# mathisbot/homomorph-rust

Measured on AMD Instinct MI355X. Metric: homomorphic u32 ops/sec (add, mul) at d=dp=tau=128; 1/2/4/8 MI355X, higher is better.
Workload: dtype u32

## Files before the change

homomorph-rust_amd/csrc/adder.hip:

```cpp
#include <hip/hip_runtime.h>

#include "dev_common.h"

namespace hm {


__device__ __forceinline__ uint32_t limb_off(const Bounds &B, uint32_t i) {
    uint32_t o = 0;
    for (uint32_t j = 0; j < i; ++j) o += cap_of(B.b[j]);
    return o;
}

__device__ __forceinline__ uint64_t checked_limb(uint64_t v, uint32_t d, uint32_t bnd, uint32_t k, bool &bad) {
    const uint32_t nl = d / 64 + 1;
    if (d > bnd) {
        bad = true;
        return 0;
    }
    if (k >= nl) {
        bad |= v != 0;
        return 0;
    }
    if (k == nl - 1) {
        const uint32_t top = d % 64;
        const uint64_t keep = (~0ull) >> (63 - top);
        bad |= (v & ~keep) != 0;
        v &= keep;
        if (d > 0 && !((v >> top) & 1ull)) bad = true;
    }
    return v;
}

__device__ __forceinline__ void stage_ab(const uint64_t *__restrict__ pa, const uint32_t *__restrict__ da,
                                         const Bounds &BA, const uint64_t *__restrict__ pb,
                                         const uint32_t *__restrict__ db, const Bounds &BB, uint32_t i0,
                                         uint32_t nb, uint32_t *Al, uint32_t cntA, uint32_t *nAl,
                                         uint32_t *Bl, uint32_t cntB, uint32_t *nBl, uint32_t *tb,
                                         int *status, uint32_t bmask = ~0u) {
    const uint32_t lane = (uint32_t)lane_id();
    i0 = rfl(i0), nb = rfl(nb);
    pa += limb_off(BA, i0), pb += limb_off(BB, i0);
    da += i0, db += i0;
    uint32_t dga = 0, dgb = 0;
    if (lane < nb) dga = da[lane], dgb = db[lane];
    uint32_t tota = 0, totb = 0, vba = 0, vea = 0, vbb = 0, veb = 0;
    for (uint32_t t = 0; t < nb; ++t) {
        const uint32_t j = (i0 + t) & bmask;
        const uint32_t ba = BA.b[j], bb = BB.b[j];
        tota += cap_of(ba), totb += cap_of(bb);
        if (lane == t) vba = ba, vea = tota, vbb = bb, veb = totb;
    }
    const uint64_t fa = lane < tota ? pa[lane] : 0ull, fb = lane < totb ? pb[lane] : 0ull;
    uint32_t *bnda = tb, *enda = tb + nb, *bndb = tb + 2 * nb, *endb = tb + 3 * nb;
    if (lane < nb) {
        bnda[lane] = vba, enda[lane] = vea, bndb[lane] = vbb, endb[lane] = veb;
        nAl[lane] = dga, nBl[lane] = dgb;
    }
    for (uint32_t k = lane; k < nb * cntA; k += kWave) Al[k] = 0u;
    for (uint32_t k = lane; k < nb * cntB; k += kWave) Bl[k] = 0u;
    wsync();
    bool bad = false;
    auto one = [&](const uint64_t *src, uint64_t first, uint32_t total, const uint32_t *bnd,
                   const uint32_t *ends, const uint32_t *deg, uint32_t *dst, uint32_t cnt) {
        uint32_t t = 0, lo = 0, hi = nb ? ends[0] : 0;
        for (uint32_t g = lane; g < total; g += kWave) {
            while (g >= hi) ++t, lo = hi, hi = ends[t];
            const uint32_t k = g - lo;
            const uint64_t v = checked_limb(g == lane ? first : src[g], deg[t], bnd[t], k, bad);
            dst[t * cnt + 2 * k] = (uint32_t)v;
            dst[t * cnt + 2 * k + 1] = (uint32_t)(v >> 32);
        }
    };
    one(pa, fa, tota, bnda, enda, nAl, Al, cntA);
    one(pb, fb, totb, bndb, endb, nBl, Bl, cntB);
    if (__any(bad) && lane == 0) flag(status, HM_ERR_BAD_INPUT);
    wsync();
    if (lane < nb) {
        const uint32_t d1 = nAl[lane], d2 = nBl[lane];
        uint32_t n1 = d1 / 32 + 1, n2 = d2 / 32 + 1;
        if (d1 > bnda[lane] || (d1 == 0 && !(Al[lane * cntA] & 1u))) n1 = 0;
        if (d2 > bndb[lane] || (d2 == 0 && !(Bl[lane * cntB] & 1u))) n2 = 0;
        nAl[lane] = n1, nBl[lane] = n2;
    }
}

template <int NB, int NAB, bool TOP1 = false, bool MULTI = false>
__global__ void __launch_bounds__(256) add_prep_kernel(AddArgs A) {
    extern __shared__ uint32_t lds[];
    const uint32_t wave = rfl(threadIdx.x >> 6);
    const uint64_t gw = (uint64_t)blockIdx.x * (blockDim.x >> 6) + wave;
    const int lane = lane_id();
    const uint32_t L = A.nbits;
    uint64_t e;
    uint32_t bpw, i0, nmine;
    if constexpr (MULTI) {
        e = gw * A.vpw;
        if (e >= A.n) return;
        bpw = A.vpw * L;
        i0 = 0;
        nmine = (uint32_t)min((uint64_t)A.vpw, A.n - e) * L;
    } else {
        e = gw / A.wpv;
        const uint32_t part = (uint32_t)(gw % A.wpv);
        if (e >= A.n) return;
        bpw = (L + A.wpv - 1) / A.wpv;
        i0 = min(L, part * bpw), nmine = min(L, i0 + bpw) - i0;
    }
    auto val_of = [&](uint32_t t) -> uint32_t { return MULTI ? t >> A.lgL : 0u; };
    auto bit_of = [&](uint32_t t) -> uint32_t { return MULTI ? t & (L - 1) : i0 + t; };
    uint32_t *Ls = lds + (size_t)wave * A.prep_lds;
    uint32_t *Al = Ls, *Bl = Al + bpw * A.cntA, *Xl = Bl + bpw * A.cntB;
    uint32_t *ABl = Xl + bpw * A.cntX, *Pl = ABl + bpw * A.cntAB;
    uint32_t *nAl = Pl + bpw * A.cntP, *nBl = nAl + bpw, *dAB = nBl + bpw, *dP = dAB + bpw;
    const size_t oP = (size_t)L * A.cntAB, oDA = oP + (size_t)L * A.cntP, oDP = oDA + L, oX = oDP + L;
    uint32_t *ws = A.ws + e * A.ws_stride;
    auto wsv = [&](uint32_t t) { return MULTI ? ws + (size_t)val_of(t) * A.ws_stride : ws; };
    const uint64_t *pa = A.a.limbs + e * A.a.stride, *pb = A.b.limbs + e * A.b.stride;
    const uint32_t *da = A.a.degree + e * L, *db = A.b.degree + e * L;

    stage_ab(pa, da, A.ab, pb, db, A.bb, i0, nmine, Al, A.cntA, nAl, Bl, A.cntB, nBl, dAB, A.status,
             MULTI ? L - 1 : ~0u);
    for (uint32_t k = lane; k < 2 * bpw; k += kWave) dAB[k] = 0u;
    wsync();
    const uint32_t nprod = MULTI ? nmine : min(nmine, (L - 1) - min(i0, L - 1));
    auto has_prod = [&](uint32_t t) { return !MULTI || bit_of(t) + 1 < L; };

    for (uint32_t f = lane; f < nmine * A.cntX; f += kWave) {
        const uint32_t t = f / A.cntX, m = f % A.cntX, i = bit_of(t);
        const int na = (int)nAl[t], nb = (int)nBl[t];
        const uint32_t x = ((int)m < na ? Al[t * A.cntA + m] : 0u) ^
                           ((int)m < nb ? Bl[t * A.cntB + m] : 0u);
        Xl[t * A.cntX + m] = x;
        wsv(t)[oX + (size_t)i * A.cntX + m] = x;
    }

    const uint32_t cq = A.cntX - (TOP1 ? 1u : 0u);
    const uint32_t qt = A.cntX - 1;
    auto top_rows = [&](uint32_t cnt, auto &&len, auto &&set, const uint32_t *src, uint32_t scnt,
                        uint32_t *dst, uint32_t dcnt) {
        const uint32_t dt = kWave / cnt, dk = kWave % cnt;
        uint32_t t = (uint32_t)lane / cnt, k = (uint32_t)lane % cnt;
        for (uint32_t f0 = 0; f0 < nprod * cnt; f0 += kWave) {
            if (t < nprod && has_prod(t) && k < len(t) && set(t))
                atomicXor(&dst[t * dcnt + qt + k], src[t * scnt + k]);
            t += dt, k += dk;
            if (k >= cnt) k -= cnt, ++t;
        }
    };
    auto for_rows = [&](auto &&row) {
        const uint32_t dt = kWave / cq, dq = kWave % cq;
        uint32_t t = (uint32_t)lane / cq, q = (uint32_t)lane % cq;
        for (uint32_t f0 = 0; f0 < nprod * cq; f0 += kWave) {
            if (t < nprod && has_prod(t)) row(t, q);
            t += dt, q += dq;
            if (q >= cq) q -= cq, ++t;
        }
    };
    for (uint32_t k = lane; k < nprod * A.cntAB; k += kWave) ABl[k] = 0u;
    for (uint32_t k = lane; k < nprod * A.cntP; k += kWave) Pl[k] = 0u;
    wsync();
    for_rows([&](uint32_t t, uint32_t q) {
        if ((int)q < (int)nAl[t]) {
            if constexpr (NB > 0) {
                if (nBl[t]) clmul_row_xor_fixed<NB>(Al[t * A.cntA + q], Bl + t * NB, ABl + t * NAB + q);
            } else {
                clmul_row_xor(Al[t * A.cntA + q], Bl + t * A.cntB, (int)nBl[t], ABl + t * A.cntAB + q);
            }
        }
    });
    if constexpr (TOP1)
        top_rows(A.cntB, [&](uint32_t t) { return nBl[t]; }, [&](uint32_t t) { return nAl[t] == A.cntX; },
                 Bl, A.cntB, ABl, A.cntAB);
    wsync();
    for (uint32_t f = lane; f < nprod * A.cntAB; f += kWave) {
        const uint32_t t = f / A.cntAB, m = f % A.cntAB;
        const uint32_t w = ABl[f];
        if (has_prod(t)) wsv(t)[(size_t)bit_of(t) * A.cntAB + m] = w;
        if (w) atomicMax(&dAB[t], m * 32 + 32 - __builtin_clz(w));
    }
    wsync();
    for_rows([&](uint32_t t, uint32_t q) {
        const int nx = max((int)nAl[t], (int)nBl[t]);
        if ((int)q < nx) {
            if constexpr (NAB > 0) {
                if (dAB[t]) clmul_row_xor_fixed<NAB>(Xl[t * A.cntX + q], ABl + t * NAB, Pl + t * A.cntP + q);
            } else {
                clmul_row_xor(Xl[t * A.cntX + q], ABl + t * A.cntAB, bitwords((int)dAB[t]),
                              Pl + t * A.cntP + q);
            }
        }
    });
    if constexpr (TOP1)
        top_rows(A.cntAB, [&](uint32_t t) { return (uint32_t)bitwords((int)dAB[t]); },
                 [&](uint32_t t) { return (Xl[t * A.cntX + qt] & 1u) != 0; }, ABl, A.cntAB, Pl, A.cntP);
    wsync();
    for (uint32_t f = lane; f < nprod * A.cntP; f += kWave) {
        const uint32_t t = f / A.cntP, m = f % A.cntP;
        const uint32_t w = Pl[f] ^ (m < A.cntX ? Xl[t * A.cntX + m] : 0u);
        if (has_prod(t)) wsv(t)[oP + (size_t)bit_of(t) * A.cntP + m] = w;
        if (w) atomicMax(&dP[t], m * 32 + 32 - __builtin_clz(w));
    }
    wsync();
    for (uint32_t t = lane; t < nprod; t += kWave) {
        if (!has_prod(t)) continue;
        const uint32_t i = bit_of(t);
        wsv(t)[oDA + i] = dAB[t];
        wsv(t)[oDP + i] = dP[t];
    }
}

template <int CAP>
__global__ void __launch_bounds__(256) add_prep_uniform_kernel(AddArgs A) {
    constexpr uint32_t kBound = 64u * (CAP - 1);
    constexpr uint32_t cA = 2 * CAP, cX = 2 * CAP - 1, cAB = 4 * CAP - 3, cP = 6 * CAP - 5;
    constexpr uint32_t cq = cX - 1, qt = cX - 1;
    extern __shared__ uint32_t lds[];
    const uint32_t wave = rfl(threadIdx.x >> 6);
    const uint64_t gw = (uint64_t)blockIdx.x * (blockDim.x >> 6) + wave;
    const uint32_t lane = (uint32_t)lane_id();
    const uint32_t L = A.nbits;
    uint64_t e;
    uint32_t part;
    if ((gw >> 32) == 0)
        e = (uint32_t)gw / A.wpv, part = (uint32_t)gw % A.wpv;
    else
        e = gw / A.wpv, part = (uint32_t)(gw % A.wpv);
    if (e >= A.n) return;
    const uint32_t bpw = (L + A.wpv - 1) / A.wpv;
    const uint32_t i0 = rfl(min(L, part * bpw)), nmine = rfl(min(L, i0 + bpw) - i0);
    const uint32_t nprod = rfl(min(nmine, (L - 1) - min(i0, L - 1)));
    auto lanes = [&](uint32_t n, auto &&body) {
        for (uint32_t f0 = 0; f0 < n; f0 += kWave)
            if (f0 + lane < n) body(f0 + lane);
    };
    uint32_t *Ls = lds + (size_t)wave * A.prep_lds;
    uint32_t *Al = Ls, *Bl = Al + bpw * cA, *Xl = Bl + bpw * cA;
    uint32_t *ABl = Xl + bpw * cX, *Pl = ABl + bpw * cAB;
    uint32_t *nAl = Pl + bpw * cP, *nBl = nAl + bpw, *nXl = nBl + bpw, *nABl = nXl + bpw;
    uint32_t *dXl = nABl + bpw;
    const size_t oP = (size_t)L * cAB, oDA = oP + (size_t)L * cP, oDP = oDA + L, oX = oDP + L;
    uint32_t *ws = A.ws + e * A.ws_stride;
    const uint64_t *pa = A.a.limbs + e * A.a.stride + (size_t)i0 * CAP;
    const uint64_t *pb = A.b.limbs + e * A.b.stride + (size_t)i0 * CAP;
    const uint32_t *da = A.a.degree + e * L + i0, *db = A.b.degree + e * L + i0;

    uint32_t dga = 0, dgb = 0;
    if (lane < nmine) dga = da[lane], dgb = db[lane];
    const uint32_t tot = nmine * CAP;
    uint64_t fa[2], fb[2];
#pragma unroll
    for (uint32_t j = 0; j < 2; ++j) {
        const uint32_t g = lane + j * kWave;
        fa[j] = g < tot ? pa[g] : 0ull, fb[j] = g < tot ? pb[g] : 0ull;
    }
    lanes(nprod * cAB, [&](uint32_t f) { ABl[f] = 0u; });
    constexpr uint32_t cPz = cP - cX;
    lanes(nprod * cPz, [&](uint32_t f) { Pl[f / cPz * cP + cX + f % cPz] = 0u; });
    if (lane < nmine) nAl[lane] = dga, nBl[lane] = dgb, dXl[lane] = 0u;
    wsync();
    bool bad = false;
    auto stage = [&](uint32_t g, uint64_t va, uint64_t vb) {
        const uint32_t t = g / CAP, k = g % CAP;
        va = checked_limb(va, nAl[t], kBound, k, bad);
        vb = checked_limb(vb, nBl[t], kBound, k, bad);
        *(uint2 *)(Al + t * cA + 2 * k) = make_uint2((uint32_t)va, (uint32_t)(va >> 32));
        *(uint2 *)(Bl + t * cA + 2 * k) = make_uint2((uint32_t)vb, (uint32_t)(vb >> 32));
        const uint64_t x = va ^ vb;
        const uint32_t xl = (uint32_t)x, xh = (uint32_t)(x >> 32);
        uint32_t *xs = Xl + t * cX + 2 * k, *xg = ws + oX + (size_t)(i0 + t) * cX + 2 * k;
        uint32_t *xp = Pl + t * cP + 2 * k;
        const bool prod = t < nprod;
        xs[0] = xl, xg[0] = xl;
        if (prod) xp[0] = xl;
        if (k + 1 < CAP) {
            xs[1] = xh, xg[1] = xh;
            if (prod) xp[1] = xh;
        }
        if (x) atomicMax(&dXl[t], 64 * k + 64 - (uint32_t)__builtin_clzll(x));
    };
#pragma unroll
    for (uint32_t j = 0; j < 2; ++j)
        if (lane + j * kWave < tot) stage(lane + j * kWave, fa[j], fb[j]);
    for (uint32_t g0 = 2 * kWave; g0 < tot; g0 += kWave)
        if (g0 + lane < tot) stage(g0 + lane, pa[g0 + lane], pb[g0 + lane]);
    if (__any(bad) && lane == 0) flag(A.status, HM_ERR_BAD_INPUT);
    wsync();
    if (lane < nmine) {
        uint32_t a1 = dga + 1, b1 = dgb + 1;
        if (dga > kBound || (dga == 0 && !(Al[lane * cA] & 1u))) a1 = 0;
        if (dgb > kBound || (dgb == 0 && !(Bl[lane * cA] & 1u))) b1 = 0;
        const uint32_t x1 = dXl[lane];
        const uint32_t ab1 = a1 && b1 ? a1 + b1 - 1 : 0u;
        const uint32_t p1 = !x1 ? 0u : !ab1 ? x1 : x1 + ab1 - 1;
        nAl[lane] = (uint32_t)bitwords((int)a1), nBl[lane] = (uint32_t)bitwords((int)b1);
        nXl[lane] = (uint32_t)bitwords((int)x1), nABl[lane] = (uint32_t)bitwords((int)ab1);
        if (lane < nprod) ws[oDA + i0 + lane] = ab1, ws[oDP + i0 + lane] = p1;
    }
    wsync();
    lanes(nprod * cq, [&](uint32_t f) {
        const uint32_t t = f / cq, q = f % cq;
        if (q < nAl[t]) clmul_row_xor(Al[t * cA + q], Bl + t * cA, (int)nBl[t], ABl + t * cAB + q);
    });
    lanes(nprod * cA, [&](uint32_t f) {
        const uint32_t t = f / cA, k = f % cA;
        if (k < nBl[t] && nAl[t] == cX) atomicXor(&ABl[t * cAB + qt + k], Bl[f]);
    });
    wsync();
    uint32_t *wsab = ws + (size_t)i0 * cAB, *wsp = ws + oP + (size_t)i0 * cP;
    lanes(nprod * cAB, [&](uint32_t f) {
        const uint32_t t = f / cAB, k = f % cAB;
        const uint32_t w = ABl[f];
        wsab[f] = w;
        if (k < nABl[t] && (Xl[t * cX + qt] & 1u)) atomicXor(&Pl[t * cP + qt + k], w);
    });
    lanes(nprod * cq, [&](uint32_t f) {
        const uint32_t t = f / cq, q = f % cq;
        if (q < nXl[t]) clmul_row_xor(Xl[t * cX + q], ABl + t * cAB, (int)nABl[t], Pl + t * cP + q);
    });
    wsync();
    lanes(nprod * cP, [&](uint32_t f) { wsp[f] = Pl[f]; });
}

__device__ __forceinline__ int store_sum_bit(const uint64_t *pa, uint32_t dga, const uint64_t *pb, uint32_t dgb,
                             const uint32_t *C, int nc, uint64_t *__restrict__ dst, uint32_t bound,
                             uint32_t *deg_out, int *status) {
    const int lane = lane_id();
    const int cap = (int)cap_of(bound);
    const int nla = (int)(dga >> 6) + 1, nlb = (int)(dgb >> 6) + 1;
    const uint64_t ma = (~0ull) >> (63 - (dga & 63)), mb = (~0ull) >> (63 - (dgb & 63));
    const int total = max(max(cap, max(nla, nlb)), (nc + 1) / 2);
    int ldeg = -1;
    for (int g = lane; g < total; g += kWave) {
        uint64_t v = 0;
        if (g < nla) v ^= g == nla - 1 ? (pa[g] & ma) : pa[g];
        if (g < nlb) v ^= g == nlb - 1 ? (pb[g] & mb) : pb[g];
        const int w = 2 * g;
        const uint32_t lo = w < nc ? C[w] : 0u, hi = w + 1 < nc ? C[w + 1] : 0u;
        v ^= (uint64_t)lo | ((uint64_t)hi << 32);
        if (g < cap) dst[g] = v;
        if (v) ldeg = g * 64 + 63 - __builtin_clzll(v);
    }
    const int deg = wave_max_i32(ldeg);
    if (lane == 0) {
        if (deg > (int)bound) flag(status, HM_ERR_CAPACITY);
        *deg_out = (uint32_t)max(deg, 0);
    }
    return deg;
}

template <int WMAX, bool PAD>
__global__ void __launch_bounds__(256) add_chain_kernel(AddArgs A) {
    kt_start(A.kt);
    extern __shared__ uint32_t lds[];
    const int wave = (int)rfl(threadIdx.x >> 6);
    const uint64_t e = (uint64_t)blockIdx.x * (blockDim.x >> 6) + wave;
    if (e >= A.n) {
        kt_finish(A.kt);
        return;
    }
    const int lane = lane_id();
    const uint32_t L = A.nbits;
    uint32_t *Ls = lds + (size_t)wave * A.chain_lds;
    uint32_t *C = Ls + kHalo, *Cn = C + A.cw + kHalo;
    uint32_t *Pl = Cn + A.cw;
    const uint32_t *ws = A.ws + e * A.ws_stride;
    const uint32_t *ABg = ws, *Pg = ws + (size_t)L * A.cntAB;
    const uint32_t *degABg = Pg + (size_t)L * A.cntP, *degPg = degABg + L;
    const uint64_t *pa = A.a.limbs + e * A.a.stride, *pb = A.b.limbs + e * A.b.stride;
    uint64_t *po = A.out.limbs + e * A.out.stride;
    const uint32_t *da = A.a.degree + e * L, *db = A.b.degree + e * L;
    uint32_t *dout = A.out.degree + e * L;

    const uint32_t ncarry = 2 * (A.cw + kHalo);
    for (uint32_t k = lane; k < ncarry; k += kWave) Ls[k] = 0u;
    for (uint32_t k = lane; k < (L - 1) * A.cntP; k += kWave) Pl[k] = Pg[k];
    wsync();
    int nc = 0;
    uint32_t offa = 0, offb = 0, offo = 0;
    for (uint32_t i = 0; i < L; ++i) {
        store_sum_bit(pa + offa, rfl(da[i]), pb + offb, rfl(db[i]), C, nc, po + offo, A.ob.b[i],
                      dout + i, A.status);
        if (i + 1 < L) {
            const int np = bitwords((int)degPg[i]), nab = bitwords((int)degABg[i]);
            int nout;
            nc = words_of(wave_mul<kQBig, WMAX, PAD>(Pl + (size_t)i * A.cntP, np, C, nc,
                                                     ABg + (size_t)i * A.cntAB, nab, Cn, &nout));
            wsync();
            uint32_t *t = C;
            C = Cn;
            Cn = t;
        }
        offa += cap_of(A.ab.b[i]);
        offb += cap_of(A.bb.b[i]);
        offo += cap_of(A.ob.b[i]);
    }
    kt_finish(A.kt);
}

template <int WMAX>
__global__ void __launch_bounds__(256) add_chain_staged_kernel(AddArgs A) {
    kt_start(A.kt);
    extern __shared__ uint32_t lds[];
    const int wave = (int)rfl(threadIdx.x >> 6);
    const uint64_t e = (uint64_t)blockIdx.x * (blockDim.x >> 6) + wave;
    if (e >= A.n) {
        kt_finish(A.kt);
        return;
    }
    const int lane = lane_id();
    const uint32_t L = A.nbits;
    uint32_t *Ls = lds + (size_t)wave * A.chain_lds;
    uint32_t *C = Ls + kHalo;
    uint32_t *Pl = C + A.cw, *ABl = Pl + (size_t)(L - 1) * A.cntP;
    uint32_t *Xl = ABl + (size_t)(L - 1) * A.cntAB, *dPl = Xl + (size_t)L * A.cntX, *dABl = dPl + L;
    const uint32_t *ws = A.ws + e * A.ws_stride;
    const uint32_t *ABg = ws, *Pg = ws + (size_t)L * A.cntAB;
    const uint32_t *degABg = Pg + (size_t)L * A.cntP, *degPg = degABg + L, *Xg = degPg + L;
    uint64_t *po = A.out.limbs + e * A.out.stride;
    uint32_t *dout = A.out.degree + e * L;

    for (uint32_t k = lane; k < kHalo + A.cw; k += kWave) Ls[k] = 0u;
    for (uint32_t k = lane; k < (L - 1) * A.cntP; k += kWave) Pl[k] = Pg[k];
    for (uint32_t k = lane; k < (L - 1) * A.cntAB; k += kWave) ABl[k] = ABg[k];
    for (uint32_t k = lane; k < L * A.cntX; k += kWave) Xl[k] = Xg[k];
    for (uint32_t k = lane; k < L; k += kWave) dPl[k] = degPg[k], dABl[k] = degABg[k];
    wsync();
    int nc = 0;
    uint32_t offo = 0;
    for (uint32_t i = 0; i < L; ++i) {
        store_sum_x(Xl + (size_t)i * A.cntX, (int)A.cntX, C, nc, po + offo, A.ob.b[i], dout + i,
                    A.status);
        if (i + 1 < L) {
            const int np = bitwords((int)rfl(dPl[i])), nab = bitwords((int)rfl(dABl[i]));
            int nout;
            wsync();
            nc = words_of(wave_mul<kQBig, WMAX, true>(Pl + (size_t)i * A.cntP, np, C, nc,
                                                      ABl + (size_t)i * A.cntAB, nab, C, &nout));
            wsync();
        }
        offo += cap_of(A.ob.b[i]);
    }
    kt_finish(A.kt);
}

int launch_add_prep(const AddArgs &a, void *stream) {
    if (a.n == 0) return 0;
    const uint64_t waves = a.vpw > 1 ? (a.n + a.vpw - 1) / a.vpw : a.n * a.wpv;
    const uint64_t blocks = (waves + 3) / 4;
    const size_t lds = (size_t)a.prep_lds * 4 * 4;
#ifndef HM_PREP_FIXED
#define HM_PREP_FIXED 0
#endif
    if (a.ucap == 5 && a.vpw <= 1)
        hipLaunchKernelGGL((add_prep_uniform_kernel<5>), dim3((unsigned)blocks), dim3(256), lds, (hipStream_t)stream, a);
    else if (a.ucap)
        return -1;
    else if (a.vpw > 1 && a.top1)
        hipLaunchKernelGGL((add_prep_kernel<0, 0, true, true>), dim3((unsigned)blocks), dim3(256), lds, (hipStream_t)stream, a);
    else if (a.vpw > 1)
        hipLaunchKernelGGL((add_prep_kernel<0, 0, false, true>), dim3((unsigned)blocks), dim3(256), lds, (hipStream_t)stream, a);
    else if (a.top1)
        hipLaunchKernelGGL((add_prep_kernel<0, 0, true>), dim3((unsigned)blocks), dim3(256), lds, (hipStream_t)stream, a);
    else if (HM_PREP_FIXED && a.cntB == 10 && a.cntAB == 17)
        hipLaunchKernelGGL((add_prep_kernel<10, 17>), dim3((unsigned)blocks), dim3(256), lds, (hipStream_t)stream, a);
    else if (HM_PREP_FIXED && a.cntB == 6 && a.cntAB == 9)
        hipLaunchKernelGGL((add_prep_kernel<6, 9>), dim3((unsigned)blocks), dim3(256), lds, (hipStream_t)stream, a);
    else if (HM_PREP_FIXED && a.cntB == 18 && a.cntAB == 33)
        hipLaunchKernelGGL((add_prep_kernel<18, 33>), dim3((unsigned)blocks), dim3(256), lds, (hipStream_t)stream, a);
    else
        hipLaunchKernelGGL((add_prep_kernel<0, 0>), dim3((unsigned)blocks), dim3(256), lds, (hipStream_t)stream, a);
    return hipGetLastError() == hipSuccess ? 0 : -1;
}

AddArgs add_args_slice(const AddArgs &a, uint64_t e0, uint64_t n) {
    AddArgs s = a;
    s.a.limbs += e0 * a.a.stride, s.a.degree += e0 * a.a.dstride;
    s.b.limbs += e0 * a.b.stride, s.b.degree += e0 * a.b.dstride;
    s.out.limbs += e0 * a.out.stride, s.out.degree += e0 * a.out.dstride;
    s.ws += e0 * a.ws_stride;
    s.n = n;
    return s;
}

int launch_add(const AddArgs &a, void *stream) {
    if (a.n == 0) return 0;
    if (launch_add_prep(a, stream)) return -1;
    return a.mfma ? launch_add_chain_mfma(a, stream) : launch_add_chain_valu(a, stream);
}

int launch_add_chain_valu(const AddArgs &a, void *stream) {
    const int wpb = kAddWavesPerBlock;
    const uint64_t blocks = (a.n + wpb - 1) / wpb;
    const size_t lds = (size_t)a.chain_lds * 4 * wpb;
    const uint32_t need = (a.max_prod_words + 63) / 64;
    const bool pad = a.pad != 0;
#define HM_LAUNCH_ADD(WM)                                                                         \
    do {                                                                                          \
        if (a.staged)                                                                             \
            hipLaunchKernelGGL((add_chain_staged_kernel<WM>), dim3((unsigned)blocks),             \
                               dim3(64 * wpb), lds, (hipStream_t)stream, a);                      \
        else if (pad)                                                                             \
            hipLaunchKernelGGL((add_chain_kernel<WM, true>), dim3((unsigned)blocks),              \
                               dim3(64 * wpb), lds, (hipStream_t)stream, a);                      \
        else                                                                                      \
            hipLaunchKernelGGL((add_chain_kernel<WM, false>), dim3((unsigned)blocks),             \
                               dim3(64 * wpb), lds, (hipStream_t)stream, a);                      \
    } while (0)
    if (need <= 4) HM_LAUNCH_ADD(4);
    else if (need <= 8) HM_LAUNCH_ADD(8);
    else if (need <= 12) HM_LAUNCH_ADD(12);
    else if (need <= 16) HM_LAUNCH_ADD(16);
    else HM_LAUNCH_ADD(24);
#undef HM_LAUNCH_ADD
    return hipGetLastError() == hipSuccess ? 0 : -1;
}

}
```

homomorph-rust_amd/csrc/dev_common.h:

```cpp
#pragma once
#include <hip/hip_runtime.h>

#include "engine.h"
#include "gf2_wave.h"

namespace hm {

__device__ __forceinline__ void flag(int *status, int code) {
    if (status) atomicCAS(status, 0, code);
}

__device__ __forceinline__ void wsync() {
    __builtin_amdgcn_fence(__ATOMIC_RELEASE, "wavefront");
    __builtin_amdgcn_wave_barrier();
    __builtin_amdgcn_fence(__ATOMIC_ACQUIRE, "wavefront");
}
__device__ __forceinline__ void gsync() {
    __builtin_amdgcn_fence(__ATOMIC_RELEASE, "workgroup");
    __builtin_amdgcn_wave_barrier();
    __builtin_amdgcn_fence(__ATOMIC_ACQUIRE, "workgroup");
}


__device__ __forceinline__ void arg_to_lds(const uint32_t (&a)[HM_MAX_BITS], uint32_t n, uint32_t *lds) {
    static_assert(HM_MAX_BITS % 16 == 0, "whole 16-entry chunks");
    n = rfl(n);
    const bool l0 = (threadIdx.x & 63u) == 0;
    for (uint32_t c = 0; c < n; c += 16) {
        uint32_t v[16];
#pragma unroll
        for (int j = 0; j < 16; ++j) v[j] = a[c + j];
        if (l0) {
            uint4 *d = (uint4 *)(lds + c);
#pragma unroll
            for (int q = 0; q < 4; ++q) d[q] = make_uint4(v[4 * q], v[4 * q + 1], v[4 * q + 2], v[4 * q + 3]);
        }
    }
}

__device__ __forceinline__ int load_bit(const uint64_t *__restrict__ src, uint32_t deg, uint32_t bound,
                        uint32_t *__restrict__ dst, int *status) {
    const int lane = lane_id();
    if (deg > bound) {
        if (lane == 0) flag(status, HM_ERR_BAD_INPUT);
        return 0;
    }
    const int nl = (int)(deg / 64) + 1;
    const int cap = (int)(bound / 64) + 1;
    const uint32_t tb = deg % 64;
    bool bad = false;
    for (int g = lane; g < cap; g += kWave) {
        uint64_t v = src[g];
        if (g >= nl) {
            bad |= v != 0;
            continue;
        }
        if (g == nl - 1) {
            const uint64_t keep = (~0ull) >> (63 - tb);
            bad |= (v & ~keep) != 0;
            v &= keep;
            if (deg > 0 && !((v >> tb) & 1ull)) bad = true;
        }
        dst[2 * g] = (uint32_t)v;
        dst[2 * g + 1] = (uint32_t)(v >> 32);
    }
    if (__any(bad) && lane == 0) flag(status, HM_ERR_BAD_INPUT);
    if (deg == 0) {
        const uint32_t w0 = rfl((uint32_t)src[0]);
        if (!(w0 & 1u)) return 0;
    }
    return (int)(deg / 32) + 1;
}

__device__ __forceinline__ int store_xor_bit(const uint32_t *X, int nx, const uint32_t *C, int nc,
                             uint64_t *__restrict__ dst, uint32_t bound, uint32_t *deg_out,
                             int *status) {
    const int lane = lane_id();
    const int cap = (int)cap_of(bound);
    const int n = max(nx, nc);
    const int total = max(cap, (n + 1) / 2);
    int ldeg = -1;
    for (int g = lane; g < total; g += kWave) {
        const int w = 2 * g;
        uint32_t lo = (w < nx ? X[w] : 0u) ^ (w < nc ? C[w] : 0u);
        uint32_t hi = (w + 1 < nx ? X[w + 1] : 0u) ^ (w + 1 < nc ? C[w + 1] : 0u);
        uint64_t v = (uint64_t)lo | ((uint64_t)hi << 32);
        if (g < cap) dst[g] = v;
        if (v) ldeg = g * 64 + 63 - __builtin_clzll(v);
    }
    const int deg = wave_max_i32(ldeg);
    if (lane == 0) {
        if (deg > (int)bound) flag(status, HM_ERR_CAPACITY);
        *deg_out = (uint32_t)max(deg, 0);
    }
    return deg;
}

struct WaveSlice {
    uint64_t e;
    uint32_t *lds;
    bool live;
};
__device__ __forceinline__ WaveSlice wave_slice(uint32_t *lds, uint32_t lds_per_wave, uint64_t n) {
    const int wave = (int)rfl(threadIdx.x >> 6);
    const uint64_t e = (uint64_t)blockIdx.x * (blockDim.x >> 6) + wave;
    return {e, lds + (size_t)wave * lds_per_wave, e < n};
}

struct BitReader {
    const uint64_t *limbs;
    const uint32_t *degree;
    uint32_t off = 0;
    int *status;
    __device__ __forceinline__ BitReader(const BatchArg &x, uint64_t e, int *status)
        : limbs(x.limbs + e * x.stride), degree(x.degree + e * x.dstride), status(status) {}
    __device__ __forceinline__ int load(uint32_t i, uint32_t bound, uint32_t *dst) {
        const int n = load_bit(limbs + off, rfl(degree[i]), bound, dst, status);
        off += cap_of(bound);
        return n;
    }
    __device__ __forceinline__ int load_down(uint32_t i, uint32_t bound, uint32_t *dst) {
        off -= cap_of(bound);
        return load_bit(limbs + off, rfl(degree[i]), bound, dst, status);
    }
};
struct BitWriter {
    uint64_t *limbs;
    uint32_t *degree;
    uint32_t off = 0;
    int *status;
    __device__ __forceinline__ BitWriter(const BatchArg &x, uint64_t e, int *status)
        : limbs(x.limbs + e * x.stride), degree(x.degree + e * x.dstride), status(status) {}
    __device__ __forceinline__ void store(uint32_t i, uint32_t bound, const uint32_t *X, int nx,
                                          const uint32_t *C = nullptr, int nc = 0) {
        store_xor_bit(X, nx, C, nc, limbs + off, bound, degree + i, status);
        off += cap_of(bound);
    }
};

__device__ __forceinline__ int store_sum_x(const uint32_t *X, int nx, const uint32_t *C, int nc,
                           uint64_t *__restrict__ dst, uint32_t bound, uint32_t *deg_out,
                           int *status) {
    const int lane = lane_id();
    const int cap = (int)cap_of(bound);
    const int total = max(cap, (max(nx, nc) + 1) / 2);
    int ldeg = -1;
    for (int g = lane; g < total; g += kWave) {
        const int w = 2 * g;
        const uint32_t lo = (w < nx ? X[w] : 0u) ^ (w < nc ? C[w] : 0u);
        const uint32_t hi = (w + 1 < nx ? X[w + 1] : 0u) ^ (w + 1 < nc ? C[w + 1] : 0u);
        const uint64_t v = (uint64_t)lo | ((uint64_t)hi << 32);
        if (g < cap) dst[g] = v;
        if (v) ldeg = g * 64 + 63 - __builtin_clzll(v);
    }
    const int deg = wave_max_i32(ldeg);
    if (lane == 0) {
        if (deg > (int)bound) flag(status, HM_ERR_CAPACITY);
        *deg_out = (uint32_t)max(deg, 0);
    }
    return deg;
}

__device__ __forceinline__ int words_of(int deg) { return deg >= 0 ? nwords(deg) : 0; }

__device__ __forceinline__ int store_xor3_bit(const uint32_t *Aw, int na, const uint32_t *Bw, int nb,
                              const uint32_t *C, int nc, uint64_t *__restrict__ dst,
                              uint32_t bound, uint32_t *deg_out, int *status) {
    const int lane = lane_id();
    const int cap = (int)cap_of(bound);
    const int n = max(max(na, nb), nc);
    const int total = max(cap, (n + 1) / 2);
    int ldeg = -1;
    for (int g = lane; g < total; g += kWave) {
        const int w = 2 * g;
        uint32_t lo = (w < na ? Aw[w] : 0u) ^ (w < nb ? Bw[w] : 0u) ^ (w < nc ? C[w] : 0u);
        uint32_t hi = (w + 1 < na ? Aw[w + 1] : 0u) ^ (w + 1 < nb ? Bw[w + 1] : 0u) ^
                      (w + 1 < nc ? C[w + 1] : 0u);
        uint64_t v = (uint64_t)lo | ((uint64_t)hi << 32);
        if (g < cap) dst[g] = v;
        if (v) ldeg = g * 64 + 63 - __builtin_clzll(v);
    }
    const int deg = wave_max_i32(ldeg);
    if (lane == 0) {
        if (deg > (int)bound) flag(status, HM_ERR_CAPACITY);
        *deg_out = (uint32_t)max(deg, 0);
    }
    return deg;
}

constexpr int kQSmall = 10;
constexpr int kQBig = 25;

struct Holey {
    uint32_t h[4];
    __device__ __forceinline__ explicit Holey(uint32_t v) {
#pragma unroll
        for (int a = 0; a < 4; ++a) h[a] = v & (0x11111111u << a);
    }
};

__device__ __forceinline__ void holey_acc(uint32_t z[4], const Holey &U, const Holey &V1,
                                          const Holey &V0) {
#pragma unroll
    for (int c = 0; c < 4; ++c) {
        uint32_t lo[4], hi[4];
#pragma unroll
        for (int a = 0; a < 4; ++a) {
            const int b = (c - a) & 3;
            lo[a] = U.h[a] * V1.h[b];
            hi[a] = __umulhi(U.h[a], V0.h[b]);
        }
        z[c] = __builtin_amdgcn_bitop3_b32(__builtin_amdgcn_bitop3_b32(z[c], lo[0], lo[1], 0x96),
                                           __builtin_amdgcn_bitop3_b32(lo[2], lo[3], hi[0], 0x96),
                                           __builtin_amdgcn_bitop3_b32(hi[1], hi[2], hi[3], 0x96), 0x96);
    }
}

__device__ __forceinline__ uint32_t xor4(uint32_t a, uint32_t b, uint32_t c, uint32_t d) {
    return __builtin_amdgcn_bitop3_b32(a, b, c, 0x96) ^ d;
}

__device__ __forceinline__ uint32_t holey_fold(const uint32_t z[4]) {
    return (z[0] & 0x11111111u) | (z[1] & 0x22222222u) | (z[2] & 0x44444444u) |
           (z[3] & 0x88888888u);
}

__device__ __forceinline__ uint32_t clmul_word(const uint32_t *__restrict__ pu, int nu,
                                               const uint32_t *__restrict__ pv, int nv, int m) {
    uint32_t z[4] = {0u, 0u, 0u, 0u};
    const int qlo = max(0, m - nv), qhi = min(nu - 1, m);
    if (qlo > qhi) return 0u;
    int k = m - qlo;
    Holey V1(k < nv ? pv[k] : 0u);
    for (int q = qlo; q <= qhi; ++q, --k) {
        const Holey V0((k >= 1 && k - 1 < nv) ? pv[k - 1] : 0u);
        holey_acc(z, Holey(pu[q]), V1, V0);
        V1 = V0;
    }
    return holey_fold(z);
}

__device__ __forceinline__ void clmul_row_xor(uint32_t u, const uint32_t *__restrict__ pv, int nv,
                                              uint32_t *out) {
    const Holey U(u);
    uint32_t hiprev = 0u;
#ifndef HM_CLMUL_PEEL
#define HM_CLMUL_PEEL 1
#endif
    if (HM_CLMUL_PEEL) {
        if (nv <= 0) return;
        uint32_t vnext = pv[0];
        for (int k = 0; k < nv; ++k) {
            const Holey V(vnext);
            vnext = pv[min(k + 1, nv - 1)];
            uint32_t zl[4], zh[4];
#pragma unroll
            for (int c = 0; c < 4; ++c) {
                uint64_t p[4];
#pragma unroll
                for (int a = 0; a < 4; ++a) p[a] = (uint64_t)U.h[a] * V.h[(c - a) & 3];
                zl[c] = xor4((uint32_t)p[0], (uint32_t)p[1], (uint32_t)p[2], (uint32_t)p[3]);
                zh[c] = xor4((uint32_t)(p[0] >> 32), (uint32_t)(p[1] >> 32), (uint32_t)(p[2] >> 32),
                             (uint32_t)(p[3] >> 32));
            }
            atomicXor(&out[k], holey_fold(zl) ^ hiprev);
            hiprev = holey_fold(zh);
        }
        if (hiprev) atomicXor(&out[nv], hiprev);
        return;
    }
    uint32_t vnext = nv > 0 ? pv[0] : 0u;
    for (int k = 0; k <= nv; ++k) {
        uint32_t lo = 0u, hi = 0u;
        if (k < nv) {
            const Holey V(vnext);
            vnext = k + 1 < nv ? pv[k + 1] : 0u;
            uint32_t zl[4], zh[4];
#pragma unroll
            for (int c = 0; c < 4; ++c) {
                uint64_t p[4];
#pragma unroll
                for (int a = 0; a < 4; ++a) p[a] = (uint64_t)U.h[a] * V.h[(c - a) & 3];
                zl[c] = xor4((uint32_t)p[0], (uint32_t)p[1], (uint32_t)p[2], (uint32_t)p[3]);
                zh[c] = xor4((uint32_t)(p[0] >> 32), (uint32_t)(p[1] >> 32), (uint32_t)(p[2] >> 32),
                             (uint32_t)(p[3] >> 32));
            }
            lo = holey_fold(zl), hi = holey_fold(zh);
        }
        const uint32_t w = lo ^ hiprev;
        if (w) atomicXor(&out[k], w);
        hiprev = hi;
    }
}

template <int NV>
__device__ __forceinline__ void clmul_row_xor_fixed(uint32_t u, const uint32_t *__restrict__ pv,
                                                    uint32_t *out) {
    const Holey U(u);
    uint32_t v[NV];
#pragma unroll
    for (int k = 0; k < NV; ++k) v[k] = pv[k];
    uint32_t hiprev = 0u;
#pragma unroll
    for (int k = 0; k < NV; ++k) {
        const Holey V(v[k]);
        uint32_t zl[4], zh[4];
#pragma unroll
        for (int c = 0; c < 4; ++c) {
            uint64_t p[4];
#pragma unroll
            for (int a = 0; a < 4; ++a) p[a] = (uint64_t)U.h[a] * V.h[(c - a) & 3];
            zl[c] = xor4((uint32_t)p[0], (uint32_t)p[1], (uint32_t)p[2], (uint32_t)p[3]);
            zh[c] = xor4((uint32_t)(p[0] >> 32), (uint32_t)(p[1] >> 32), (uint32_t)(p[2] >> 32),
                         (uint32_t)(p[3] >> 32));
        }
        atomicXor(&out[k], holey_fold(zl) ^ hiprev);
        hiprev = holey_fold(zh);
    }
    if (hiprev) atomicXor(&out[NV], hiprev);
}

__device__ __forceinline__ uint32_t kt_wave() {
    return (blockIdx.x * ((blockDim.x + 63u) >> 6) + (threadIdx.x >> 6)) & (kTimerWaves - 1);
}
__device__ __forceinline__ void kt_start(const KTimer &k) {
    if (k.t0 && (threadIdx.x & 63u) == 0)
        __hip_atomic_fetch_min(&k.t0[kt_wave()], (unsigned long long)wall_clock64(),
                               __ATOMIC_RELAXED, __HIP_MEMORY_SCOPE_AGENT);
}
__device__ __forceinline__ void kt_finish(const KTimer &k) {
    if (k.t1 && (threadIdx.x & 63u) == 0)
        __hip_atomic_fetch_max(&k.t1[kt_wave()], (unsigned long long)wall_clock64(),
                               __ATOMIC_RELAXED, __HIP_MEMORY_SCOPE_AGENT);
}

__device__ __forceinline__ int bitwords(int degp1) { return degp1 ? ((degp1 - 1) >> 5) + 1 : 0; }

}
```

Before: 9.828 million.

## Pair holey-multiply products and peel monic top words from GF(2) clmul rows

Restructures the carry-less multiply core so some pairs of holey sub-products are summed with one integer add before extraction. Static checks confirm no 4-bit field overflows, cutting the XOR count, and folding uses bitop3 bit-select with masks held opaque in VGPRs. In the polynomial product kernel, the known-monic leading word of each operand is handled with direct XORs of the other operand's words instead of full clmul rows, shortening row lengths. This adds constexpr bookkeeping and relies on the leading-word-equals-one invariant for correctness.

```diff
diff --git a/homomorph-rust_amd/csrc/adder.hip b/homomorph-rust_amd/csrc/adder.hip
--- a/homomorph-rust_amd/csrc/adder.hip
+++ b/homomorph-rust_amd/csrc/adder.hip
@@ -299,23 +299,31 @@
     wsync();
     lanes(nprod * cq, [&](uint32_t f) {
         const uint32_t t = f / cq, q = f % cq;
-        if (q < nAl[t]) clmul_row_xor(Al[t * cA + q], Bl + t * cA, (int)nBl[t], ABl + t * cAB + q);
+        if (q < nAl[t])
+            clmul_row_xor(Al[t * cA + q], Bl + t * cA, (int)min(nBl[t], qt), ABl + t * cAB + q);
     });
     lanes(nprod * cA, [&](uint32_t f) {
         const uint32_t t = f / cA, k = f % cA;
-        if (k < nBl[t] && nAl[t] == cX) atomicXor(&ABl[t * cAB + qt + k], Bl[f]);
+        const uint32_t w = (nAl[t] == cX && k < cX ? Bl[f] : 0u) ^ (nBl[t] == cX && k < qt ? Al[f] : 0u);
+        if (w) atomicXor(&ABl[t * cAB + qt + k], w);
     });
     wsync();
+    constexpr uint32_t qtab = cAB - 1;
     uint32_t *wsab = ws + (size_t)i0 * cAB, *wsp = ws + oP + (size_t)i0 * cP;
     lanes(nprod * cAB, [&](uint32_t f) {
         const uint32_t t = f / cAB, k = f % cAB;
         const uint32_t w = ABl[f];
         wsab[f] = w;
         if (k < nABl[t] && (Xl[t * cX + qt] & 1u)) atomicXor(&Pl[t * cP + qt + k], w);
+        if (k < qt && nABl[t] == cAB) {
+            const uint32_t x = Xl[t * cX + k];
+            if (x) atomicXor(&Pl[t * cP + qtab + k], x);
+        }
     });
     lanes(nprod * cq, [&](uint32_t f) {
         const uint32_t t = f / cq, q = f % cq;
-        if (q < nXl[t]) clmul_row_xor(Xl[t * cX + q], ABl + t * cAB, (int)nABl[t], Pl + t * cP + q);
+        if (q < nXl[t])
+            clmul_row_xor(Xl[t * cX + q], ABl + t * cAB, (int)min(nABl[t], qtab), Pl + t * cP + q);
     });
     wsync();
     lanes(nprod * cP, [&](uint32_t f) { wsp[f] = Pl[f]; });
diff --git a/homomorph-rust_amd/csrc/dev_common.h b/homomorph-rust_amd/csrc/dev_common.h
--- a/homomorph-rust_amd/csrc/dev_common.h
+++ b/homomorph-rust_amd/csrc/dev_common.h
@@ -240,82 +240,118 @@
     return holey_fold(z);
 }
 
+struct HoleyTerm {
+    int a0, b0, a1, b1;
+};
+constexpr int kHoleyTerms = 12;
+constexpr int kHoleyClass[5] = {0, 3, 5, 8, 12};
+constexpr HoleyTerm holey_term(int t) {
+    constexpr HoleyTerm T[kHoleyTerms] = {
+        {0, 0, 1, 3}, {2, 2, -1, -1}, {3, 1, -1, -1},
+        {0, 1, 2, 3}, {1, 0, 3, 2},
+        {3, 3, 0, 2}, {1, 1, -1, -1}, {2, 0, -1, -1},
+        {0, 3, -1, -1}, {1, 2, -1, -1}, {2, 1, -1, -1}, {3, 0, -1, -1}
+    };
+    return T[t];
+}
+constexpr int holey_pairs_at(int a, int b, int p) {
+    int n = 0;
+    for (int i = 0; i < 8; ++i)
+        for (int j = 0; j < 8; ++j) n += a + 4 * i + b + 4 * j == p;
+    return n;
+}
+constexpr bool holey_terms_ok() {
+    int seen[4][4] = {};
+    for (int c = 0; c < 4; ++c)
+        for (int t = kHoleyClass[c]; t < kHoleyClass[c + 1]; ++t) {
+            const HoleyTerm T = holey_term(t);
+            if (T.a0 < 0 || T.a0 > 3 || T.b0 < 0 || T.b0 > 3 || ((T.a0 + T.b0) & 3) != c) return false;
+            ++seen[T.a0][T.b0];
+            const bool two = T.a1 >= 0;
+            if (two) {
+                if (T.a1 > 3 || T.b1 < 0 || T.b1 > 3 || ((T.a1 + T.b1) & 3) != c) return false;
+                ++seen[T.a1][T.b1];
+            }
+            for (int p = 0; p < 72; ++p)
+                if (holey_pairs_at(T.a0, T.b0, p) + (two ? holey_pairs_at(T.a1, T.b1, p) : 0) > 15)
+                    return false;
+        }
+    for (int a = 0; a < 4; ++a)
+        for (int b = 0; b < 4; ++b)
+            if (seen[a][b] != 1) return false;
+    return true;
+}
+static_assert(holey_terms_ok(), "holey_term: a summed pair overflows its 4-bit field, or a product is missing");
+
+__device__ __forceinline__ uint32_t vgpr_opaque(uint32_t v) {
+    asm volatile("" : "+v"(v));
+    return v;
+}
+struct HoleyMasks {
+    uint32_t m0, m2, m01;
+    __device__ __forceinline__ HoleyMasks()
+        : m0(vgpr_opaque(0x11111111u)), m2(vgpr_opaque(0x44444444u)), m01(vgpr_opaque(0x33333333u)) {}
+};
+__device__ __forceinline__ uint32_t bitsel(uint32_t m, uint32_t a, uint32_t b) {
+    return __builtin_amdgcn_bitop3_b32(m, a, b, 0xCA);
+}
+__device__ __forceinline__ uint32_t xor3(uint32_t a, uint32_t b, uint32_t c) {
+    return __builtin_amdgcn_bitop3_b32(a, b, c, 0x96);
+}
+
+struct ClmulWords {
+    uint32_t lo, hi;
+};
+__device__ __forceinline__ ClmulWords holey_product(const Holey &U, const Holey &V, const HoleyMasks &M) {
+    static_assert(kHoleyClass[1] == 3 && kHoleyClass[2] == 5 && kHoleyClass[3] == 8 && kHoleyClass[4] == 12,
+                  "the XORs below are written for 3, 2, 3 and 4 terms");
+    uint32_t l[kHoleyTerms], h[kHoleyTerms];
+#pragma unroll
+    for (int t = 0; t < kHoleyTerms; ++t) {
+        const HoleyTerm T = holey_term(t);
+        uint64_t p = (uint64_t)U.h[T.a0] * V.h[T.b0];
+        if (T.a1 >= 0) p += (uint64_t)U.h[T.a1] * V.h[T.b1];
+        l[t] = (uint32_t)p, h[t] = (uint32_t)(p >> 32);
+    }
+    auto fold = [&](const uint32_t (&z)[kHoleyTerms]) {
+        const uint32_t z0 = xor3(z[0], z[1], z[2]), z1 = z[3] ^ z[4], z2 = xor3(z[5], z[6], z[7]);
+        const uint32_t z3 = xor4(z[8], z[9], z[10], z[11]);
+        return bitsel(M.m01, bitsel(M.m0, z0, z1), bitsel(M.m2, z2, z3));
+    };
+    return {fold(l), fold(h)};
+}
+
 __device__ __forceinline__ void clmul_row_xor(uint32_t u, const uint32_t *__restrict__ pv, int nv,
                                               uint32_t *out) {
+    if (nv <= 0) return;
     const Holey U(u);
+    const HoleyMasks M;
     uint32_t hiprev = 0u;
-#ifndef HM_CLMUL_PEEL
-#define HM_CLMUL_PEEL 1
-#endif
-    if (HM_CLMUL_PEEL) {
-        if (nv <= 0) return;
-        uint32_t vnext = pv[0];
-        for (int k = 0; k < nv; ++k) {
-            const Holey V(vnext);
-            vnext = pv[min(k + 1, nv - 1)];
-            uint32_t zl[4], zh[4];
-#pragma unroll
-            for (int c = 0; c < 4; ++c) {
-                uint64_t p[4];
-#pragma unroll
-                for (int a = 0; a < 4; ++a) p[a] = (uint64_t)U.h[a] * V.h[(c - a) & 3];
-                zl[c] = xor4((uint32_t)p[0], (uint32_t)p[1], (uint32_t)p[2], (uint32_t)p[3]);
-                zh[c] = xor4((uint32_t)(p[0] >> 32), (uint32_t)(p[1] >> 32), (uint32_t)(p[2] >> 32),
-                             (uint32_t)(p[3] >> 32));
-            }
-            atomicXor(&out[k], holey_fold(zl) ^ hiprev);
-            hiprev = holey_fold(zh);
-        }
-        if (hiprev) atomicXor(&out[nv], hiprev);
-        return;
-    }
-    uint32_t vnext = nv > 0 ? pv[0] : 0u;
-    for (int k = 0; k <= nv; ++k) {
-        uint32_t lo = 0u, hi = 0u;
-        if (k < nv) {
-            const Holey V(vnext);
-            vnext = k + 1 < nv ? pv[k + 1] : 0u;
-            uint32_t zl[4], zh[4];
-#pragma unroll
-            for (int c = 0; c < 4; ++c) {
-                uint64_t p[4];
-#pragma unroll
-                for (int a = 0; a < 4; ++a) p[a] = (uint64_t)U.h[a] * V.h[(c - a) & 3];
-                zl[c] = xor4((uint32_t)p[0], (uint32_t)p[1], (uint32_t)p[2], (uint32_t)p[3]);
-                zh[c] = xor4((uint32_t)(p[0] >> 32), (uint32_t)(p[1] >> 32), (uint32_t)(p[2] >> 32),
-                             (uint32_t)(p[3] >> 32));
-            }
-            lo = holey_fold(zl), hi = holey_fold(zh);
-        }
-        const uint32_t w = lo ^ hiprev;
-        if (w) atomicXor(&out[k], w);
-        hiprev = hi;
-    }
+    uint32_t vnext = pv[0];
+    for (int k = 0; k < nv; ++k) {
+        const Holey V(vnext);
+        vnext = pv[min(k + 1, nv - 1)];
+        const ClmulWords w = holey_product(U, V, M);
+        atomicXor(&out[k], w.lo ^ hiprev);
+        hiprev = w.hi;
+    }
+    if (hiprev) atomicXor(&out[nv], hiprev);
 }
 
 template <int NV>
 __device__ __forceinline__ void clmul_row_xor_fixed(uint32_t u, const uint32_t *__restrict__ pv,
                                                     uint32_t *out) {
     const Holey U(u);
+    const HoleyMasks M;
     uint32_t v[NV];
 #pragma unroll
     for (int k = 0; k < NV; ++k) v[k] = pv[k];
     uint32_t hiprev = 0u;
 #pragma unroll
     for (int k = 0; k < NV; ++k) {
-        const Holey V(v[k]);
-        uint32_t zl[4], zh[4];
-#pragma unroll
-        for (int c = 0; c < 4; ++c) {
-            uint64_t p[4];
-#pragma unroll
-            for (int a = 0; a < 4; ++a) p[a] = (uint64_t)U.h[a] * V.h[(c - a) & 3];
-            zl[c] = xor4((uint32_t)p[0], (uint32_t)p[1], (uint32_t)p[2], (uint32_t)p[3]);
-            zh[c] = xor4((uint32_t)(p[0] >> 32), (uint32_t)(p[1] >> 32), (uint32_t)(p[2] >> 32),
-                         (uint32_t)(p[3] >> 32));
-        }
-        atomicXor(&out[k], holey_fold(zl) ^ hiprev);
-        hiprev = holey_fold(zh);
+        const ClmulWords w = holey_product(U, Holey(v[k]), M);
+        atomicXor(&out[k], w.lo ^ hiprev);
+        hiprev = w.hi;
     }
     if (hiprev) atomicXor(&out[NV], hiprev);
 }
```

Measured after the change: 9.870 million, median of 6. About the same (+0.4%).
